# opensensor/thingino-accel

Measured on AMD Instinct MI355X. Metric: images/sec yolov5s_int8 640x640 batch256, higher is better.
Workload: dtype int8

## Files before the change

thingino-accel_amd/csrc/hip/conv_i8.hip:

```cpp
#include "conv_i8_common.hpp"

#ifndef I8M_ABL
#define I8M_ABL 0
#endif
template <int BPX, int BN, int STAGES, int KS = 1, int NW = 4>
__global__ __launch_bounds__(NW * 64) void conv_i8_mfma(const mhip_conv_i8_t p, const long total_pix, const int k64,
                                                         const int8_t *__restrict__ zeros, const unsigned noc,
                                                         const unsigned nblk, const int lg_inc, const unsigned kw_magic,
                                                         const fastdiv_t dhw, const fastdiv_t dow, const int bufmode,
                                                         const unsigned in_bytes) {
    ANAT_BEGIN();
    const bool POW2 = lg_inc >= 0;
    const bool masked = p.kh * p.kw <= 32;
    constexpr int SLICE = (BPX + BN) * BK;
    constexpr int STAGE = KS * SLICE;
    constexpr int NWN = BN == 128 ? 2 : 1;
    constexpr int NWM = NW / NWN;
    constexpr int WPX = BPX / NWM / 16;
    constexpr int WOC = BN / NWN / 16;
    constexpr int XROWS = BPX / NW;
    constexpr int XI = XROWS / 16;
    constexpr int LW = (BN / 16 + NW - 1) / NW;
    constexpr int L = XI + LW;
    static_assert(XI >= 1 && XROWS % 16 == 0, "every wave fetches whole 16-row pieces of the pixel tile");
// ... 713 lines not shown
        if (c < 1.0 || c > 2147483647.0) continue;
        volatile float prod = (float)(int)c * a;
        if (prod == quirk) return 0;
    }
    return 1;
}

extern "C" int mhip_conv_i8_small_c(int in_c, int kw, int out_c) { return in_c <= 4 && kw <= 8 && out_c <= 64; }

extern "C" void mhip_conv_i8_pack_geom(int in_c, int kw, int out_c, int *row_pad, int *oc_pad, int *c_eff) {
    const int small = mhip_conv_i8_small_c(in_c, kw, out_c);
    if (row_pad) *row_pad = small ? 32 : (kw * in_c + 15) & ~15;
    if (oc_pad) *oc_pad = (out_c + 31) & ~31;
    if (c_eff) *c_eff = small ? 4 : in_c;
}

static tune_t g_tune;
static int env_int(const char *name, int dflt) {
    const char *e = getenv(name);
    return e ? atoi(e) : dflt;
}
const tune_t &conv_i8_tune_state() {
    if (!g_tune.init) {
        g_tune.persist = env_int("MARS_HIP_PERSIST", 1);
        g_tune.persist_stages = env_int("MARS_HIP_PSTAGES", 2);
        g_tune.persist_maxk = env_int("MARS_HIP_PERSIST_MAXK", 8);
        g_tune.persist_slots = env_int("MARS_HIP_PSLOTS", 0);
        g_tune.stages = env_int("MARS_HIP_STAGES", 0);
        g_tune.bpx = env_int("MARS_HIP_BPX", 0);
        g_tune.variant = env_int("MARS_HIP_VARIANT", 0);
        g_tune.bufmode = env_int("MARS_HIP_BUFMODE", 1);
        g_tune.wres = env_int("MARS_HIP_WRES", 3);
        g_tune.rgb_direct = env_int("MARS_HIP_RGB_DIRECT", 1);
        g_tune.small_batch = env_int("MARS_HIP_SMALL_BATCH", 1);
        g_tune.rows = env_int("MARS_HIP_ROWS", 1);
        g_tune.few_wgs = env_int("MARS_HIP_FEW_WGS", 256);
        g_tune.patch_ring = env_int("MARS_HIP_PATCH_RING", 0);
        g_tune.patch_lds_kb = env_int("MARS_HIP_PATCH_LDS_KB", 80);
        g_tune.init = 1;
    }
    return g_tune;
}
static inline const tune_t &tune() { return conv_i8_tune_state(); }
static int tune_access(const char *key, int value, int *get) {
    (void)conv_i8_tune_state();
    struct { const char *k; int *v; } tab[] = {{"persist", &g_tune.persist}, {"persist_stages", &g_tune.persist_stages},
                                               {"persist_maxk", &g_tune.persist_maxk}, {"persist_slots", &g_tune.persist_slots}, {"wres", &g_tune.wres}, {"rgb_direct", &g_tune.rgb_direct}, {"small_batch", &g_tune.small_batch},
                                               {"rows", &g_tune.rows}, {"few_wgs", &g_tune.few_wgs}, {"patch_ring", &g_tune.patch_ring}, {"patch_lds_kb", &g_tune.patch_lds_kb}, {"stages", &g_tune.stages}, {"bpx", &g_tune.bpx}, {"variant", &g_tune.variant}, {"bufmode", &g_tune.bufmode}};
    for (auto &e : tab)
        if (key && !strcmp(key, e.k)) {
            if (get) *get = *e.v;
            else *e.v = value;
            return 0;
        }
    return -1;
}
extern "C" int mhip_conv_i8_tune(const char *key, int value) { return tune_access(key, value, nullptr); }
extern "C" int mhip_conv_i8_tune_get(const char *key, int *value) { return value ? tune_access(key, 0, value) : -1; }

static int buf_mode(const mhip_conv_i8_t *p, int k64) {
    if (!tune().bufmode) return 0;
    return p->in_c >= 64 && (p->in_c & (p->in_c - 1)) == 0 && p->kh * p->kw <= 32 && (long)p->kh * p->kw * (p->kw - 1) < 65536 &&
           in_extent_bytes(p) <= 0x7fffffffL && (long)p->oc_pad * k64 <= 0x7fffffffL;
}

template <int BPX, int BN, int STAGES, int KS = 1, int NW = 4>
static int launch_mfma(const mhip_conv_i8_t *p, long total_pix, int k64) {
    const unsigned npt = (unsigned)((total_pix + BPX - 1) / BPX), noc = (unsigned)(p->oc_pad / BN);
    const unsigned nblk = npt * noc;
    const int nks = k64 / BK, nst = nks / KS, used = nst < STAGES ? nst : STAGES;
    if (KS > 1 && (nks % KS) != 0) return -1;
    size_t ring = (size_t)used * KS * (BPX + BN) * BK, tile = (size_t)BPX * (BN + OPAD);
    const size_t lds = BPX * 8 + LUTB + (ring > tile ? ring : tile);
    if (lds > 64 * 1024) {
        static bool attr = false;
        if (!attr && hipFuncSetAttribute((const void *)conv_i8_mfma<BPX, BN, STAGES, KS, NW>, hipFuncAttributeMaxDynamicSharedMemorySize,
                                         (int)(BPX * 8 + LUTB + (size_t)STAGES * KS * (BPX + BN) * BK)) != hipSuccess)
            return mhip_check(hipErrorUnknown, "conv_i8_mfma LDS attribute");
        attr = true;
    }
    int lg = -1;
    if ((p->in_c & (p->in_c - 1)) == 0 && (long)p->kh * p->kw * (p->kw - 1) < 65536) {
        lg = 0;
        while ((1 << lg) < p->in_c) lg++;
    }
    const unsigned magic = ((65536u + (unsigned)p->kw - 1u) / (unsigned)p->kw);
    hipLaunchKernelGGL((conv_i8_mfma<BPX, BN, STAGES, KS, NW>), dim3(nblk), dim3(NW * 64), lds, mhip_stream_native(), *p, total_pix,
                       k64, (const int8_t *)mhip_zero_page(), noc, nblk, lg, magic,
                       make_fastdiv((unsigned)(p->out_h * p->out_w)), make_fastdiv((unsigned)p->out_w),
                       lg >= 0 ? buf_mode(p, k64) : 0, (unsigned)in_extent_bytes(p));
    return mhip_check(hipGetLastError(), "conv_i8_mfma launch");
}


template <int BPX, int BN>
static size_t wres_lds(int k64) { return LUTB + 2 * (size_t)BPX * BK + (size_t)(k64 / BK) * BN * BK; }

template <int BPX, int BN, int STAGES, bool HAS_LUT, bool SEG = false, bool PAIR = false>
static int launch_persist_t(const mhip_conv_i8_t *p, long total_pix, int k64, int lg, unsigned magic,
                            const mhip_conv_i8_t *second = nullptr, int wres = 0) {
    if (BN == 16 && (p->out_c > 16 || p->oc_pad != 32 || (PAIR && (second->out_c > 16 || second->oc_pad != 32)))) return -1;
    const unsigned noc0 = BN == 16 ? 1u : (unsigned)(p->oc_pad / BN);
    const unsigned npt = (unsigned)((total_pix + BPX - 1) / BPX), noc = noc0 + (PAIR ? (BN == 16 ? 1u : (unsigned)(second->oc_pad / BN)) : 0u);
    conv_out_side_t alt;
    memset(&alt, 0, sizeof(alt));
    if (PAIR) {
        alt.out = second->out; alt.out_stride = second->out_stride; alt.w = second->w; alt.bias = second->bias;
        alt.lut = second->lut; alt.lut2 = second->lut2; alt.out_c = second->out_c; alt.relu = second->relu; alt.out_pix_stride = second->out_pix_stride;
        alt.out_ch_off = second->out_ch_off; alt.cs = second->cs;
    }
    if (PAIR) alt.out_bytes = (unsigned)persist_out_bytes(second);
    if (wres && STAGES != 2) return -1;
    const size_t lds = wres ? wres_lds<BPX, BN>(k64) : LUTB + (size_t)STAGES * (BPX + BN) * BK;
    if (wres) {
        static bool attr = false;
        if (!attr && hipFuncSetAttribute((const void *)conv_i8_persist<BPX, BN, STAGES, HAS_LUT, SEG, PAIR>,
                                         hipFuncAttributeMaxDynamicSharedMemorySize, 80 * 1024) != hipSuccess)
            return mhip_check(hipErrorUnknown, "conv_i8_persist LDS attribute");
        attr = true;
        int occ = 0, dev = 0;
        hipDeviceProp_t prop;
        if (hipOccupancyMaxActiveBlocksPerMultiprocessor(&occ, conv_i8_persist<BPX, BN, STAGES, HAS_LUT, SEG, PAIR>, NTHREADS, lds) != hipSuccess ||
            hipGetDevice(&dev) != hipSuccess || hipGetDeviceProperties(&prop, dev) != hipSuccess)
            return mhip_check(hipErrorUnknown, "conv_i8_persist occupancy query");
        unsigned g = (unsigned)((occ > 0 ? occ : 1) * prop.multiProcessorCount) / noc;
        if (tune().persist_slots > 0) g = (unsigned)tune().persist_slots / noc;
        if (g < 1) g = 1;
        if (g > npt) g = npt;
        hipLaunchKernelGGL((conv_i8_persist<BPX, BN, STAGES, HAS_LUT, SEG, PAIR>), dim3(noc * g), dim3(NTHREADS), lds,
                           mhip_stream_native(), *p, (unsigned)total_pix, k64, (const int8_t *)mhip_zero_page(), noc, npt, g, lg,
                           magic, make_fastdiv((unsigned)(p->out_h * p->out_w)), make_fastdiv((unsigned)p->out_w),
                           (unsigned)persist_out_bytes(p), alt, noc0, SEG ? 0 : buf_mode(p, k64), (unsigned)in_extent_bytes(p), 1);
        return mhip_check(hipGetLastError(), "conv_i8_persist (resident weights) launch");
    }
    static int slots = 0;
    if (!slots) {
        int occ = 0, dev = 0;
        hipDeviceProp_t prop;
        if (hipOccupancyMaxActiveBlocksPerMultiprocessor(&occ, conv_i8_persist<BPX, BN, STAGES, HAS_LUT, SEG, PAIR>, NTHREADS, lds) != hipSuccess ||
            hipGetDevice(&dev) != hipSuccess || hipGetDeviceProperties(&prop, dev) != hipSuccess)
            return mhip_check(hipErrorUnknown, "conv_i8_persist occupancy query");
        slots = (occ > 0 ? occ : 1) * prop.multiProcessorCount;
    }
    unsigned ngrp = (unsigned)(tune().persist_slots > 0 ? tune().persist_slots : 4 * slots) / noc;
    if (ngrp < 1) ngrp = 1;
    if (ngrp > npt) ngrp = npt;
    hipLaunchKernelGGL((conv_i8_persist<BPX, BN, STAGES, HAS_LUT, SEG, PAIR>), dim3(noc * ngrp), dim3(NTHREADS), lds,
                       mhip_stream_native(), *p, (unsigned)total_pix, k64, (const int8_t *)mhip_zero_page(), noc, npt, ngrp, lg,
                       magic, make_fastdiv((unsigned)(p->out_h * p->out_w)), make_fastdiv((unsigned)p->out_w),
                       (unsigned)persist_out_bytes(p), alt, noc0, SEG ? 0 : buf_mode(p, k64), (unsigned)in_extent_bytes(p), 0);
    return mhip_check(hipGetLastError(), "conv_i8_persist launch");
}

#define NVARIANTS 20
struct variant_t {
    int persist, bpx, stages, patch, ks2, w8, wres, r128, rows;
};
static int variant_code(const variant_t &v) {
    if (v.rows) return 20;
    if (v.r128) return 17 + v.r128;
    if (v.wres) return v.bpx == 256 ? 15 : 14;
    if (v.w8) return 13;
    if (v.ks2) return 12;
    if (v.patch) return v.patch == 16 ? 10 : (v.patch == 8 ? 9 : 11);
    return 1 + (v.persist ? 1 : 0) + (v.bpx == 256 ? 2 : 0) + (v.stages == 3 ? 4 : 0);
}
static variant_t variant_of(int code) {
    if (code == 20) return variant_t{0, 0, 0, 0, 0, 0, 0, 0, 1};
    if (code == 18 || code == 19) return variant_t{0, 0, 0, 0, 0, 0, 0, code - 17, 0};
    if (code == 14 || code == 15) return variant_t{1, code == 15 ? 256 : 128, 2, 0, 0, 0, 1, 0, 0};
    if (code == 13) return variant_t{0, 256, 3, 0, 0, 1, 0, 0, 0};
    if (code == 12) return variant_t{0, 128, 2, 0, 1, 0, 0, 0, 0};
    if (code >= 9 && code <= 11) return variant_t{0, 0, 0, code == 10 ? 16 : (code == 9 ? 8 : 4), 0, 0, 0, 0, 0};
    if (code > 8 || code == 6 || code == 8) return variant_t{-1, 0, 0, 0, 0, 0, 0, 0, 0};
    const int c = code - 1;
    return variant_t{c & 1, (c & 2) ? 256 : 128, (c & 4) ? 3 : 2, 0, 0, 0, 0, 0, 0};
}

static bool r128_ok(const mhip_conv_i8_t *p) {
    const int C = p->in_c;
    return C >= 128 && (C & (C - 1)) == 0 && p->oc_pad % 128 == 0 && p->kh * p->kw <= 32 && (long)p->kh * p->kw * (p->kw - 1) < 65536 &&
           p->row_pad == p->kw * C && p->nseg <= 1 && in_extent_bytes(p) <= 0x7fffffffL && (long)p->oc_pad * p->kh * p->row_pad <= 0x7fffffffL;
}
template <int BPX, int BN, int NW>
static int launch_r128_t(const mhip_conv_i8_t *p, long total_pix) {
    const int k128 = p->kh * p->row_pad;
    const unsigned npt = (unsigned)((total_pix + BPX - 1) / BPX), noc = (unsigned)(p->oc_pad / BN);
    size_t ring = 2 * (size_t)(BPX + BN) * 128, tile = (size_t)BPX * (BN + OPAD);
    const size_t lds = BPX * 8 + LUTB + (ring > tile ? ring : tile);
    static bool attr = false;
    if (!attr && hipFuncSetAttribute((const void *)conv_i8_r128<BPX, BN, NW>, hipFuncAttributeMaxDynamicSharedMemorySize, (int)lds) != hipSuccess)
        return mhip_check(hipErrorUnknown, "conv_i8_r128 LDS attribute");
    attr = true;
    int lg = 0;
    while ((1 << lg) < p->in_c) lg++;
    const unsigned magic = ((65536u + (unsigned)p->kw - 1u) / (unsigned)p->kw);
    hipLaunchKernelGGL((conv_i8_r128<BPX, BN, NW>), dim3(npt * noc), dim3(NW * 64), lds, mhip_stream_native(), *p, total_pix, k128, noc,
                       npt * noc, lg, magic, make_fastdiv((unsigned)(p->out_h * p->out_w)), make_fastdiv((unsigned)p->out_w),
                       (unsigned)in_extent_bytes(p));
    return mhip_check(hipGetLastError(), "conv_i8_r128 launch");
}
static int launch_r128(const mhip_conv_i8_t *p, long total_pix, int form) {
    if (!r128_ok(p)) return -1;
    return form == 2 ? launch_r128_t<256, 128, 8>(p, total_pix) : launch_r128_t<128, 128, 4>(p, total_pix);
}
static bool seg_valid(const mhip_conv_i8_t *p) {
    if (p->nseg < 2 || p->nseg > 4 || p->kh != 1 || p->kw != 1 || p->stride_h != 1 || p->stride_w != 1 || p->pad_top ||
        p->pad_left || p->in_h != p->out_h || p->in_w != p->out_w)
        return false;
    int c = 0;
    if (p->seg_up && ((p->out_h | p->out_w) & 1)) return false;
    if (p->seg_up >> p->nseg) return false;
    for (int i = 0; i < 4; i++) {
        if (i < p->nseg) {
            if (!p->seg_in[i] || p->seg_c[i] <= 0 || (p->seg_c[i] & 31) || p->seg_c0[i] != c) return false;
            c += p->seg_c[i];
        } else if (p->seg_c0[i] != 0x7fffffff) {
            return false;
        }
    }
    return c == p->in_c;
}
static bool persist_eligible(const mhip_conv_i8_t *p) {
    if (p->add) return false;
    return !p->out_nchw && p->safe && (p->in_c & (p->in_c - 1)) == 0 && p->kh * p->kw <= 32 &&
           (long)p->kh * p->kw * (p->kw - 1) < 65536 && persist_out_bytes(p) <= 0x7fffffffL;
}
static bool wres_default(const mhip_conv_i8_t *p, int nks, int *bpx) {
    if (!tune().wres || p->kh * p->kw != 1 || p->in_c < 64 || p->out_h * p->out_w > 6400) return false;
    const int bn = p->oc_pad % 128 == 0 ? 128 : (p->oc_pad % 64 == 0 ? 64 : 32);
    const int px = (bn == 64 && p->out_h * p->out_w >= 6400) ? 256 : 128;
    if (LUTB + 2 * (size_t)px * BK + (size_t)nks * bn * BK > 80 * 1024) return false;
    *bpx = px;
    return true;
}

static variant_t default_variant(const mhip_conv_i8_t *p, int nks) {
    variant_t v;
    v.patch = 0;
    v.ks2 = 0;
    v.w8 = 0;
    v.wres = 0;
    v.r128 = 0;
    v.rows = 0;
    int ring = 0;
    const long wg_large = ((long)p->frames * p->out_h * p->out_w + 255) / 256 * ((p->oc_pad + 127) / 128);
    const bool few = wg_large < tune().few_wgs && tune().persist && !tune().bpx && !tune().stages && tune().small_batch;
    if (few) {
        if (conv_i8_patch_ok(p, 4, &ring)) {
            v.persist = 0; v.bpx = 0; v.stages = 0; v.patch = 4;
            return v;
        }
        if (nks >= 8 && r128_ok(p)) {
            v.persist = 0; v.bpx = 0; v.stages = 0; v.r128 = 1;
            return v;
        }
        v.bpx = 128;
        v.persist = nks <= tune().persist_maxk && persist_eligible(p);
        if (((p->out_c | p->out_pix_stride | p->out_ch_off) & 15) != 0 && p->nseg <= 1) v.persist = 0;
        v.stages = v.persist ? 2 : 3;
        return v;
    }
    if (tune().persist && !tune().bpx && !tune().stages && tune().rows && p->out_w <= 20 && p->in_c >= 256 && conv_i8_rows_ok(p)) {
        v.persist = 0; v.bpx = 0; v.stages = 0; v.rows = 1;
        return v;
    }
    if (tune().persist && !tune().bpx && !tune().stages) {
        if (conv_i8_patch_ok(p, 16, &ring)) {
            v.persist = 0; v.bpx = 0; v.stages = 0; v.patch = 16;
            return v;
        }
        if (conv_i8_patch_ok(p, 8, &ring) && ring >= 2) {
            v.persist = 0; v.bpx = 0; v.stages = 0; v.patch = 8;
            return v;
        }
    }
    v.bpx = tune().bpx ? tune().bpx : ((p->oc_pad % 128 != 0 && nks <= 2) ? 256 : 128);
    v.persist = tune().persist && nks <= tune().persist_maxk && persist_eligible(p);
    if (((p->out_c | p->out_pix_stride | p->out_ch_off) & 15) != 0 && p->nseg <= 1) v.persist = 0;
    v.stages = v.persist ? 2 : (tune().stages ? tune().stages : (nks <= 4 ? 2 : 3));
    if (v.stages != 3) v.stages = 2;
    if (v.persist && v.stages == 2 && !tune().bpx && wres_default(p, nks, &v.bpx)) v.wres = 1;
    if ((!v.persist || (!v.wres && nks >= 8 && p->nseg <= 1)) && !tune().bpx && !tune().stages && p->oc_pad % 128 == 0 &&
        nks >= (tune().persist_maxk < 8 ? tune().persist_maxk + 1 : 8)) {
        v.persist = 0; v.w8 = 1; v.bpx = 256; v.stages = 3;
    }
    if (p->nseg > 1 && !v.wres && !tune().bpx && nks >= 8) v.bpx = 256;
    return v;
}

template <int BPX, int BN>
static int launch_variant_t(const mhip_conv_i8_t *p, long total_pix, int k64, const variant_t &v) {
    if (v.persist) {
        if (!persist_eligible(p)) return -1;
        int lg = 0;
        while ((1 << lg) < p->in_c) lg++;
        const unsigned magic = ((65536u + (unsigned)p->kw - 1u) / (unsigned)p->kw);
        if (v.wres && wres_lds<BPX, BN>(k64) > 80 * 1024) return -1;
        if (p->nseg > 1)
            return p->lut ? launch_persist_t<BPX, BN, 2, true, true>(p, total_pix, k64, lg, magic, nullptr, v.wres)
                          : launch_persist_t<BPX, BN, 2, false, true>(p, total_pix, k64, lg, magic, nullptr, v.wres);
        if (v.wres)
            return p->lut ? launch_persist_t<BPX, BN, 2, true>(p, total_pix, k64, lg, magic, nullptr, 1)
                          : launch_persist_t<BPX, BN, 2, false>(p, total_pix, k64, lg, magic, nullptr, 1);
        if (v.stages == 2)
            return p->lut ? launch_persist_t<BPX, BN, 2, true>(p, total_pix, k64, lg, magic)
                          : launch_persist_t<BPX, BN, 2, false>(p, total_pix, k64, lg, magic);
        return -1;
    }
    if constexpr (BN == 16) {
        return -1;
    } else {
        if (v.w8) return BN == 128 ? launch_mfma<256, 128, 3, 1, 8>(p, total_pix, k64) : -1;
        if (v.ks2) return BPX == 128 && BN >= 64 ? launch_mfma<128, (BN >= 64 ? BN : 64), 2, 2>(p, total_pix, k64) : -1;
        return v.stages == 2 ? launch_mfma<BPX, BN, 2>(p, total_pix, k64) : launch_mfma<BPX, BN, 3>(p, total_pix, k64);
    }
}
static bool bn16_ok(const mhip_conv_i8_t *p) {
    static const bool off = getenv("MARS_HIP_NO_BN16") != nullptr;
    return !off && p->out_c <= 16 && p->oc_pad == 32 && p->nseg <= 1;
}

static int launch_variant(const mhip_conv_i8_t *p, long total_pix, int k64, const variant_t &v) {
    if (v.persist < 0) return -1;
    if (v.rows) return conv_i8_launch_rows(p);
    if (v.r128) return launch_r128(p, total_pix, v.r128);
    if (v.patch) return conv_i8_launch_patch(p, k64, v.patch);
    const int bn = p->oc_pad % 128 == 0 ? 128 : (p->oc_pad % 64 == 0 ? 64 : 32);
    const bool b16 = v.persist && v.stages == 2 && bn16_ok(p);
    if (v.bpx == 256) {
        if (bn == 128) return launch_variant_t<256, 128>(p, total_pix, k64, v);
        if (bn == 64) return launch_variant_t<256, 64>(p, total_pix, k64, v);
        if (b16) return launch_variant_t<256, 16>(p, total_pix, k64, v);
        return launch_variant_t<256, 32>(p, total_pix, k64, v);
    }
    if (bn == 128) return launch_variant_t<128, 128>(p, total_pix, k64, v);
    if (bn == 64) return launch_variant_t<128, 64>(p, total_pix, k64, v);
    if (b16) return launch_variant_t<128, 16>(p, total_pix, k64, v);
    return launch_variant_t<128, 32>(p, total_pix, k64, v);
}

template <int BPX, int BN>
static int launch_pair_t(const mhip_conv_i8_t *a, const mhip_conv_i8_t *b, long total_pix, int k64, int lg, unsigned magic,
                         int wres) {
    if (a->nseg > 1) return -2;
    return launch_persist_t<BPX, BN, 2, true, false, true>(a, total_pix, k64, lg, magic, b, wres);
}
extern "C" int mhip_conv_i8_pair(const mhip_conv_i8_t *a, const mhip_conv_i8_t *b) {
    if (!a || !b || !tune().persist || tune().variant) return -2;
    if (a->in != b->in || a->in_stride != b->in_stride || a->frames != b->frames || a->in_h != b->in_h || a->in_w != b->in_w ||
        a->in_c != b->in_c || a->out_h != b->out_h || a->out_w != b->out_w || a->kh != b->kh || a->kw != b->kw ||
        a->stride_h != b->stride_h || a->stride_w != b->stride_w || a->pad_top != b->pad_top || a->pad_left != b->pad_left ||
        a->row_pad != b->row_pad || a->nseg != b->nseg || a->seg_up != b->seg_up || !a->lut || !b->lut || a->add || b->add ||
        a->out_nchw || b->out_nchw)
        return -2;
    for (int i = 0; i < a->nseg; i++)
        if (a->seg_in[i] != b->seg_in[i] || a->seg_c[i] != b->seg_c[i] || a->seg_stride[i] != b->seg_stride[i]) return -2;
    if ((a->in_c % 16) != 0 || mhip_conv_i8_small_c(a->in_c, a->kw, a->out_c) || mhip_conv_i8_small_c(b->in_c, b->kw, b->out_c))
        return -2;
    if (a->nseg > 1 && (!seg_valid(a) || !seg_valid(b))) return -2;
    if (!persist_eligible(a) || !persist_eligible(b)) return -2;
    const int bn = a->oc_pad % 128 == 0 ? 128 : (a->oc_pad % 64 == 0 ? 64 : 32);
    const int bnb = b->oc_pad % 128 == 0 ? 128 : (b->oc_pad % 64 == 0 ? 64 : 32);
    if (bn != bnb || !mhip_zero_page()) return -2;
    const long total_pix = (long)a->frames * a->out_h * a->out_w;
    const int k64 = (a->kh * a->row_pad + BK - 1) / BK * BK, nks = k64 / BK;
    if (total_pix <= 0 || total_pix > 0x7fffffffL) return -2;
    int lg = 0;
    while ((1 << lg) < a->in_c) lg++;
    const unsigned magic = ((65536u + (unsigned)a->kw - 1u) / (unsigned)a->kw);
    const variant_t dv = default_variant(a, nks);
    const int bpx = dv.bpx ? dv.bpx : 128, wres = dv.persist && dv.wres && (tune().wres & 2);
    const bool b16 = bn16_ok(a) && bn16_ok(b);
    if (bpx == 256) {
        if (bn == 128) return launch_pair_t<256, 128>(a, b, total_pix, k64, lg, magic, wres);
        if (bn == 64) return launch_pair_t<256, 64>(a, b, total_pix, k64, lg, magic, wres);
        if (b16) return launch_pair_t<256, 16>(a, b, total_pix, k64, lg, magic, wres);
        return launch_pair_t<256, 32>(a, b, total_pix, k64, lg, magic, wres);
    }
    if (bn == 128) return launch_pair_t<128, 128>(a, b, total_pix, k64, lg, magic, wres);
    if (bn == 64) return launch_pair_t<128, 64>(a, b, total_pix, k64, lg, magic, wres);
    if (b16) return launch_pair_t<128, 16>(a, b, total_pix, k64, lg, magic, wres);
    return launch_pair_t<128, 32>(a, b, total_pix, k64, lg, magic, wres);
}

extern "C" int mhip_conv_i8_seg_ok(const mhip_conv_i8_t *p) {
    return p && (p->in_c % 16) == 0 && !mhip_conv_i8_small_c(p->in_c, p->kw, p->out_c) && seg_valid(p) && persist_eligible(p);
}

extern "C" int mhip_conv_i8_variants(const mhip_conv_i8_t *p, int *codes, int max) {
    if (!p || (p->in_c % 16) != 0 || mhip_conv_i8_small_c(p->in_c, p->kw, p->out_c)) return 0;
    const int k64 = (p->kh * p->row_pad + BK - 1) / BK * BK, nks = k64 / BK;
    int n = 0;
    if (p->pre_w) {
        const int first = conv_i8_pre_tile_rows(p);
        for (int th : {first, 16, 8, 4})
            if (th && n < max && conv_i8_patch_ok(p, th, nullptr)) {
                const int code = th == 16 ? 10 : (th == 8 ? 9 : 11);
                bool seen = false;
                for (int i = 0; i < n; i++) seen |= codes[i] == code;
                if (!seen) codes[n++] = code;
            }
        return n;
    }
    if (p->nseg > 1) {
        const int bn = p->oc_pad % 128 == 0 ? 128 : (p->oc_pad % 64 == 0 ? 64 : 32);
        const variant_t dv = default_variant(p, nks);
        const int dflt = dv.persist && dv.wres ? (dv.bpx == 256 ? 15 : 14) : (dv.bpx == 256 ? 4 : 2);
        if (n < max) codes[n++] = dflt;
        if (n < max && dflt != 2) codes[n++] = 2;
        if (n < max && dflt != 4) codes[n++] = 4;
        if (n < max && dflt != 14 && LUTB + 2 * (size_t)128 * BK + (size_t)nks * bn * BK <= 80 * 1024) codes[n++] = 14;
        if (n < max && dflt != 15 && LUTB + 2 * (size_t)256 * BK + (size_t)nks * bn * BK <= 80 * 1024) codes[n++] = 15;
        return n;
    }
    const int dflt = variant_code(default_variant(p, nks));
    if (n < max) codes[n++] = dflt;
    for (int code = 1; code <= NVARIANTS; code++) {
        const variant_t v = variant_of(code);
        if (code == dflt) continue;
        if (v.patch && !conv_i8_patch_ok(p, v.patch, nullptr)) continue;
        if (v.persist && !persist_eligible(p)) continue;
        if (v.ks2 && ((nks & 1) || nks < 4 || p->oc_pad % 64 != 0)) continue;
        if (v.w8 && (p->oc_pad % 128 != 0 || nks < 3)) continue;
        if (v.persist < 0) continue;
        if (v.r128 && !r128_ok(p)) continue;
        if (v.rows && !conv_i8_rows_ok(p)) continue;
        if (v.wres) {
            const int bn = p->oc_pad % 128 == 0 ? 128 : (p->oc_pad % 64 == 0 ? 64 : 32);
            if (LUTB + 2 * (size_t)v.bpx * BK + (size_t)nks * bn * BK > 80 * 1024) continue;
        }
        if (!v.persist && v.stages == 3 && nks <= 2) continue;
        if (n < max) codes[n++] = code;
    }
    return n;
}

template <int BN>
static int launch_generic(const mhip_conv_i8_t *p, long total_pix, int k64) {
    dim3 grid((unsigned)((total_pix + BP - 1) / BP), (unsigned)(p->oc_pad / BN));
    hipLaunchKernelGGL((conv_i8_generic<BN>), grid, dim3(NTHREADS), 0, mhip_stream_native(), *p, total_pix, k64,
                       make_fastdiv((unsigned)(p->out_h * p->out_w)));
    return mhip_check(hipGetLastError(), "conv_i8_generic launch");
}

extern "C" int mhip_conv_i8(const mhip_conv_i8_t *p) {
    if (!p || !p->in || !p->out || !p->w) return -1;
    if (p->out_pix_stride < 0 || p->out_ch_off < 0 || (p->out_nchw && (p->out_pix_stride || p->out_ch_off)) ||
        (p->out_pix_stride && p->out_pix_stride < p->out_ch_off + p->out_c))
        return -1;
    if (p->frames <= 0 || p->in_h <= 0 || p->in_w <= 0 || p->in_c <= 0 || p->out_h <= 0 || p->out_w <= 0 ||
        p->out_c <= 0 || p->kh <= 0 || p->kw <= 0 || p->stride_h < 0 || p->stride_w < 0)
        return -1;
    int row_pad, oc_pad;
    mhip_conv_i8_pack_geom(p->in_c, p->kw, p->out_c, &row_pad, &oc_pad, nullptr);
    if (row_pad != p->row_pad || oc_pad != p->oc_pad) return -1;
    if (p->add && (!p->safe || p->out_nchw || ((p->out_c | p->out_pix_stride | p->out_ch_off) & 15) || (p->in_c % 16) != 0 ||
                   mhip_conv_i8_small_c(p->in_c, p->kw, p->out_c) || p->nseg > 1))
        return -1;
    const long total_pix = (long)p->frames * p->out_h * p->out_w;
    const int k64 = (p->kh * p->row_pad + BK - 1) / BK * BK;
    if (total_pix <= 0 || total_pix > 0x7fffffffL || (total_pix + BP - 1) / BP * (oc_pad / 32) > 0x7fffffffL) return -1;
    if (p->in_planar) {
        if (p->in_planar > 4 || p->in_c != 4 || p->in_w < 4 || p->stride_h < 1 || p->stride_w < 1 || p->add || p->nseg > 1 ||
            !mhip_conv_i8_small_c(p->in_c, p->kw, p->out_c))
            return -2;
        return conv_i8_try_smallc(p, k64);
    }
    if (mhip_conv_i8_small_c(p->in_c, p->kw, p->out_c)) {
        if (p->stride_h >= 1 && p->stride_w >= 1) {
            int rc = conv_i8_try_rgb(p, k64);
            if (rc == -2) rc = conv_i8_try_smallc(p, k64);
            if (rc != -2) return rc;
        }
        if (p->add || p->nseg > 1) return -1;
        if (oc_pad % 64 == 0) return launch_generic<64>(p, total_pix, k64);
        return launch_generic<32>(p, total_pix, k64);
    }
    if (p->pre_w) {
        if (!mhip_zero_page() || !mhip_conv_i8_pre_ok(p)) return -1;
        int th = conv_i8_pre_tile_rows(p);
        const int code = p->variant ? p->variant : tune().variant;
        if (code >= 9 && code <= 11) {
            const int want = code == 10 ? 16 : (code == 9 ? 8 : 4);
            if (conv_i8_patch_ok(p, want, nullptr)) th = want;
        } else if (tune().small_batch && conv_i8_patch_ok(p, 4, nullptr) &&
                   ((long)p->frames * p->out_h * p->out_w + 255) / 256 * ((p->oc_pad + 127) / 128) < 256) {
            th = 4;
        }
        return conv_i8_launch_patch(p, k64, th);
    }
    if ((p->in_c % 16) == 0) {
        if (!mhip_zero_page()) return -1;
        const int nks = k64 / BK;
        if (p->variant < 0 || p->variant > NVARIANTS) return -1;
        int code = p->variant;
        if (p->nseg > 1) {
            if (!seg_valid(p) || !persist_eligible(p)) return -1;
            if (!code && tune().variant) {
                int codes[NVARIANTS];
                const int n = mhip_conv_i8_variants(p, codes, NVARIANTS);
                for (int i = 0; i < n; i++)
                    if (codes[i] == tune().variant) code = codes[i];
            }
            variant_t v = variant_of(code == 4 || code == 14 || code == 15 ? code : 2);
            if (!code) {
                const variant_t dv = default_variant(p, nks);
                v.bpx = dv.bpx ? dv.bpx : 128;
                v.wres = dv.persist && dv.wres;
            }
            return launch_variant(p, total_pix, k64, v);
        }
        if (!code && tune().variant) {
            int codes[NVARIANTS];
            const int n = mhip_conv_i8_variants(p, codes, NVARIANTS);
            for (int i = 0; i < n; i++)
                if (codes[i] == tune().variant) code = codes[i];
        }
        return launch_variant(p, total_pix, k64, code ? variant_of(code) : default_variant(p, nks));
    }
    if (oc_pad % 64 == 0) return launch_generic<64>(p, total_pix, k64);
    return launch_generic<32>(p, total_pix, k64);
}
```

thingino-accel_amd/csrc/hip/conv_i8_common.hpp:

```cpp
#pragma once
#include <hip/hip_runtime.h>
#include <stdint.h>
#include <stdlib.h>
#include <string.h>
#include <type_traits>

#include "../mhip.h"

extern "C" hipStream_t mhip_stream_native(void);
extern "C" int mhip_check(hipError_t e, const char *what);
extern "C" const void *mhip_zero_page(void);

typedef int v4i __attribute__((ext_vector_type(4)));
typedef int v2i __attribute__((ext_vector_type(2)));

#ifdef ANATOMY
struct anat_rec_t {
    unsigned key, wg, hwid, xcc;
    unsigned long long t[4];
};
static __device__ anat_rec_t *g_anat_buf;
static __device__ unsigned g_anat_cap;
#define ANAT_SETTER(NAME)                                                                                                    \
    extern "C" int NAME(void *buf, unsigned cap) {                                                                          \
// ... 250 lines not shown
    constexpr int ROW = BN + OPAD;
    const int lo = p.relu ? 0 : -128;
    const uint8_t *lut128 = slut + 128;
    const int chan = ocw + (lane >> 4) * (4 * WOC);
#pragma unroll
    for (int t = 0; t < WPX; t++) {
        const int prow = pxw + t * 16 + (lane & 15);
        uint32_t pk[WOC];
        int a[WOC * 4];
#pragma unroll
        for (int s = 0; s < WOC; s++)
#pragma unroll
            for (int r = 0; r < 4; r++) a[s * 4 + r] = acc[s][t][r];
        if (DIRECT && SAFE && p.add) {
            const long off = rowoff[prow];
            const bool ok = off >= 0 && oc0 + chan < p.out_c;
            uint32_t xw[WOC];
#pragma unroll
            for (int s = 0; s < WOC; s++) xw[s] = 0;
            if (ok) {
                const int8_t *x = p.add + off + oc0 + chan;
                if (WOC == 4) { const v4i t4 = *(const v4i *)x; xw[0] = t4[0]; xw[1] = t4[1]; xw[WOC > 2 ? 2 : 0] = t4[2]; xw[WOC > 3 ? 3 : 0] = t4[3]; }
                else if (WOC == 2) { const uint2 t2 = *(const uint2 *)x; xw[0] = t2.x; xw[WOC > 1 ? 1 : 0] = t2.y; }
                else xw[0] = *(const uint32_t *)x;
            }
            const add_args_t ga = {p.add_s_conv, p.add_s_other, p.add_inv};
            if (HAS_LUT && LUT0 && p.lut2) requant_pack<WOC * 4, HAS_LUT, true, LUT0, true, true>(a, p.cs, lo, lut128, pk, xw, &ga);
            else requant_pack<WOC * 4, HAS_LUT, true, LUT0, true>(a, p.cs, lo, lut128, pk, xw, &ga);
        } else {
            if (HAS_LUT && LUT0 && SAFE && p.lut2) requant_pack<WOC * 4, HAS_LUT, SAFE, LUT0, false, true>(a, p.cs, lo, lut128, pk);
            else requant_pack<WOC * 4, HAS_LUT, SAFE, LUT0>(a, p.cs, lo, lut128, pk);
        }
        if (DIRECT) {
            const long off = rowoff[prow];
            if (off >= 0 && oc0 + chan < p.out_c) {
                int8_t *d = p.out + off + oc0 + chan;
                if (WOC == 4) *(v4i *)d = (v4i){(int)pk[0], (int)pk[1], (int)pk[2], (int)pk[3]};
                else if (WOC == 2) *(uint2 *)d = make_uint2(pk[0], pk[WOC > 1 ? 1 : 0]);
                else *(uint32_t *)d = pk[0];
            }
        } else {
#pragma unroll
            for (int s = 0; s < WOC; s++) *(uint32_t *)(tile + prow * ROW + chan + s * 4) = pk[s];
        }
    }
    if (DIRECT) return;
    __syncthreads();
    const int ncols = p.out_c - oc0 < BN ? p.out_c - oc0 : BN;
    if (!p.out_nchw && ((p.out_c | p.out_pix_stride | p.out_ch_off) & 15) == 0) {
        constexpr int CPR = BN / 16;
        for (int id = tid; id < BPX * CPR; id += (int)blockDim.x) {
            const int row = id / CPR, c = id - row * CPR;
            const long off = rowoff[row];
            if (off < 0 || c * 16 >= ncols) continue;
            const int8_t *s = tile + row * ROW + c * 16;
            v4i v = {*(const int *)s, *(const int *)(s + 4), *(const int *)(s + 8), *(const int *)(s + 12)};
            *(v4i *)(p.out + off + oc0 + c * 16) = v;
        }
    } else if (!p.out_nchw) {
        constexpr int CPR = BN / 16;
        for (int id = tid; id < BPX * CPR; id += (int)blockDim.x) {
            const int row = id / CPR, c = id - row * CPR;
            const long off = rowoff[row];
            if (off < 0 || c * 16 >= ncols) continue;
            const int8_t *s = tile + row * ROW + c * 16;
            int8_t *d = p.out + off + oc0 + c * 16;
            if (c * 16 + 16 <= ncols) {
                v4i v = {*(const int *)s, *(const int *)(s + 4), *(const int *)(s + 8), *(const int *)(s + 12)};
                __builtin_memcpy(d, &v, 16);
            } else {
                const int rem = ncols - c * 16;
                int o = 0;
                if (rem & 8) { __builtin_memcpy(d, s, 8); o = 8; }
                if (rem & 4) { __builtin_memcpy(d + o, s + o, 4); o += 4; }
                if (rem & 2) { __builtin_memcpy(d + o, s + o, 2); o += 2; }
                if (rem & 1) d[o] = s[o];
            }
        }
    } else {
        for (int id = tid; id < BPX * BN; id += (int)blockDim.x) {
            const int c = id / BPX, row = id - c * BPX;
            const long off = rowoff[row];
            if (off < 0 || c >= ncols) continue;
            p.out[off + (size_t)(oc0 + c) * hw] = tile[row * ROW + c];
        }
    }
}

template <int BPX, int BN, int WPX, int WOC, bool LUT0 = false>
__device__ __forceinline__ void epilogue(const mhip_conv_i8_t &p, v4i (&acc)[WOC][WPX], int8_t *tile, const uint8_t *slut,
                                         const long *rowoff, int oc0, int pxw, int ocw, int hw) {
    const bool direct = !p.out_nchw && ((p.out_c | p.out_pix_stride | p.out_ch_off) & 15) == 0;
#define EPI(L, S, D) epilogue_t<BPX, BN, WPX, WOC, L, S, D, LUT0>(p, acc, tile, slut, rowoff, oc0, pxw, ocw, hw)
    if (direct) {
        if (p.lut) { if (p.safe) EPI(true, true, true); else EPI(true, false, true); }
        else { if (p.safe) EPI(false, true, true); else EPI(false, false, true); }
    } else {
        if (p.lut) { if (p.safe) EPI(true, true, false); else EPI(true, false, false); }
        else { if (p.safe) EPI(false, true, false); else EPI(false, false, false); }
    }
#undef EPI
}

template <int WPX, int WOC>
__device__ __forceinline__ void init_acc(const mhip_conv_i8_t &p, v4i (&acc)[WOC][WPX], int ocbase) {
    const int lane = threadIdx.x & 63;
#pragma unroll
    for (int s = 0; s < WOC; s++) {
        const v4i b = p.bias ? *(const v4i *)(p.bias + ocbase + s * 16 + (lane >> 4) * 4) : (v4i){0, 0, 0, 0};
#pragma unroll
        for (int t = 0; t < WPX; t++) acc[s][t] = b;
    }
}


struct tune_t {
    int init;
    int persist;
    int persist_stages;
    int persist_maxk;
    int persist_slots;
    int stages;
    int bpx;
    int variant;
    int bufmode;
    int small_batch;
    int rgb_direct;
    int wres;
    int few_wgs;
    int rows;
    int patch_ring;
    int patch_lds_kb;
};
const tune_t &conv_i8_tune_state();

extern "C" int mhip_conv_i8_small_c(int in_c, int kw, int out_c);

static inline long in_extent_bytes(const mhip_conv_i8_t *p) {
    return (long)(p->frames - 1) * (long)p->in_stride + (long)p->in_h * p->in_w * p->in_c;
}
static inline long persist_out_bytes(const mhip_conv_i8_t *p) {
    const long pstride = p->out_pix_stride ? p->out_pix_stride : p->out_c;
    return (long)(p->frames - 1) * (long)p->out_stride + (long)p->out_h * p->out_w * pstride;
}
static inline bool conv_i8_direct_rows(const mhip_conv_i8_t *p) {
    return !p->out_nchw && ((p->out_c | p->out_pix_stride | p->out_ch_off) & 15) == 0;
}

bool conv_i8_patch_ok(const mhip_conv_i8_t *p, int th, int *ring);
int conv_i8_launch_patch(const mhip_conv_i8_t *p, int k64, int th);
int conv_i8_pre_tile_rows(const mhip_conv_i8_t *p);
bool conv_i8_rows_ok(const mhip_conv_i8_t *p);
int conv_i8_launch_rows(const mhip_conv_i8_t *p);
int conv_i8_try_rgb(const mhip_conv_i8_t *p, int k64);
int conv_i8_try_smallc(const mhip_conv_i8_t *p, int k64);
```

thingino-accel_amd/csrc/mhip.h:

```cpp
#ifndef MHIP_H
#define MHIP_H

#include <stddef.h>
#include <stdint.h>

#ifdef __cplusplus
extern "C" {
#endif

int mhip_init(int device_hint);
void mhip_shutdown(void);
int mhip_ready(void);
int mhip_device_info(int *cu_count, int *lds_bytes, int *gfx_version, size_t *hbm_bytes);
void *mhip_stream(void);
int mhip_sync(void);
void mhip_select_aux(int on);
void mhip_select_stream(int which);
int mhip_stream_wait(int which, void *ev);
int mhip_event_sync(void *ev);
void *mhip_malloc(size_t bytes);
void mhip_free(void *p);
void *mhip_host_alloc(size_t bytes);
void mhip_host_free(void *p);
int mhip_memset_async(void *dst, int value, size_t bytes);
int mhip_h2d_async(void *dst, const void *src, size_t bytes);
int mhip_d2h_async(void *dst, const void *src, size_t bytes);
int mhip_d2d_async(void *dst, const void *src, size_t bytes);
int mhip_h2d_2d_async(void *dst, size_t dpitch, const void *src, size_t spitch, size_t row_bytes, size_t rows);
int mhip_d2h_2d_async(void *dst, size_t dpitch, const void *src, size_t spitch, size_t row_bytes, size_t rows);
void *mhip_event_create(void);
void *mhip_event_create_sync(void);
void mhip_event_destroy(void *ev);
int mhip_event_record(void *ev);
float mhip_event_elapsed_ms(void *start, void *stop);
const char *mhip_last_error(void);
int mhip_graph_begin(void);
void *mhip_graph_end(int ok);
int mhip_graph_launch(void *exec);
void mhip_graph_destroy(void *exec);

typedef struct {
    const int8_t *in;  size_t in_stride;
    int8_t *out;       size_t out_stride;
    const int8_t *w;
    const int32_t *bias;
    const uint8_t *lut;
    const uint8_t *lut2;
    const int8_t *pre_w;
    const int32_t *pre_bias;
    const uint8_t *pre_lut2;
    float pre_cs;
    const int8_t *w_rgb;
    const int8_t *w_rows;
    int frames;
    int in_h, in_w, in_c;
    int out_h, out_w, out_c;
    int kh, kw, stride_h, stride_w, pad_top, pad_left;
    int row_pad;
    int oc_pad;
    float cs;
    int relu;
    int out_nchw;
    int in_planar;
    int safe;
    int out_pix_stride;
    int out_ch_off;
    int variant;
    const int8_t *add;
    float add_s_conv, add_s_other, add_inv;
    int nseg;
    const int8_t *seg_in[4];
    size_t seg_stride[4];
    int seg_c[4], seg_c0[4];
    int seg_up;
} mhip_conv_i8_t;
int mhip_conv_i8_oc_row(int oc, int oc_pad);
int mhip_conv_i8_pre_ok(const mhip_conv_i8_t *p);
size_t mhip_conv_i8_rgb_pack(int in_c, int kh, int kw, int stride_h, int stride_w, int pad_left, int oc_pad, int k64,
                             const int8_t *packed, int8_t *out);
size_t mhip_conv_i8_rows_pack(int in_c, int kh, int kw, int stride_h, int stride_w, int oc_pad, int k64, int out_w,
                              const int8_t *packed, int8_t *out);
unsigned long mhip_conv_i8_rows_launches(void);
int mhip_conv_i8_is_safe(float cs);
int mhip_conv_i8_lut2_ok(float cs);
int mhip_conv_i8_tune(const char *key, int value);
int mhip_conv_i8_tune_get(const char *key, int *value);
int mhip_conv_i8_variants(const mhip_conv_i8_t *p, int *codes, int max);
int mhip_conv_i8_seg_ok(const mhip_conv_i8_t *p);
int mhip_conv_i8_pair(const mhip_conv_i8_t *a, const mhip_conv_i8_t *b);
int mhip_conv_i8_small_c(int in_c, int kw, int out_c);
void mhip_conv_i8_pack_geom(int in_c, int kw, int out_c, int *row_pad, int *oc_pad, int *c_eff);
int mhip_conv_i8(const mhip_conv_i8_t *p);

typedef struct {
    const float *in;  size_t in_stride;
    float *out;       size_t out_stride;
    const float *w;   const float *bias;
    const void *w_split;
    const void *w_patch;
    int frames;
    int in_h, in_w, in_c, out_h, out_w, out_c;
    int kh, kw, stride_h, stride_w, pad_top, pad_left;
    int silu;
    const float *add; size_t add_stride;
    int use_mfma;
    int k_limit;
    int k_limit_required;
    int in_rec, out_rec;
} mhip_conv_f32_t;
int mhip_conv_f32(const mhip_conv_f32_t *p);
size_t mhip_conv_f32_vcat_pack(int out_c, int in_c, int planes, const float *w, float *out);
int mhip_conv_f32_vcat_head(const mhip_conv_f32_t *p, const float *w_t, const float *const *first, const size_t *first_strides, int n_first, int run_floats);
int mhip_conv_f32_pair(const mhip_conv_f32_t *a, const mhip_conv_f32_t *b);
unsigned long mhip_conv_f32_pair_launches(void);
size_t mhip_conv_f32_split_pack(int out_c, int in_c, int kh, int kw, int stride_w, int planes, const float *w, void *out);
unsigned long mhip_conv_f32_split_launches(void);
int mhip_conv_f32_split_takes(int out_c, int in_c, int kh, int kw, int stride_h, int stride_w, int pad_left, int in_w, int out_w);
size_t mhip_conv_f32_patch_pack(int out_c, int in_c, int kh, int kw, int stride, int pad, int in_h, int in_w, int out_h, int out_w,
                                const float *w, void *out);
size_t mhip_conv_f32_patch_pack2(int out_c, int in_c, int kh, int kw, int stride, int pad, int in_h, int in_w, int out_h, int out_w,
                                 int rec, const float *w, void *out);
int mhip_conv_f32_patch_geom2(int out_c, int in_c, int kh, int kw, int stride, int pad, int in_h, int in_w, int out_h, int out_w,
                              int rec, int *outv, int cap);
unsigned long mhip_conv_f32_prec_launches(void);
unsigned long mhip_conv_f32_recin_launches(void);
int mhip_conv_f32_patch_rec_form(int out_c, int in_c, int kh, int kw, int stride, int pad, int in_h, int in_w, int out_h, int out_w);
int mhip_conv_f32_patch_geom(int out_c, int in_c, int kh, int kw, int stride, int pad, int in_h, int in_w, int out_h, int out_w,
                             int *outv, int cap);
unsigned long mhip_conv_f32_patch_launches(void);
size_t mhip_conv_f32_stem_pack(int out_c, int in_c, int kh, int kw, int stride, int pad, int in_h, int in_w, int out_h, int out_w,
                               const float *w, void *out);
unsigned long mhip_conv_f32_stem_launches(void);
int mhip_conv_f32_mode(int set);

int mhip_lut_i8(const int8_t *in, size_t in_stride, int8_t *out, size_t out_stride, int frames,
                size_t n, const uint8_t *lut_dev);
int mhip_relu_bytes(int8_t *buf, size_t stride, int frames, size_t n);
int mhip_binary_i8(int is_mul, const int8_t *a, size_t a_stride, const int8_t *b, size_t b_stride,
                   int8_t *out, size_t out_stride, int frames, size_t n, float sa, float sb, float inv_so,
                   int out_run, int out_pix_stride, int out_ch_off);
int mhip_sigmoid_f32(const float *in, size_t in_stride, float *out, size_t out_stride, int frames, size_t n);
int mhip_binary_f32(int op , const float *a, size_t a_stride, const float *b,
                    size_t b_stride, float *out, size_t out_stride, int frames, size_t n);
int mhip_relu_f32(const float *in, size_t in_stride, float *out, size_t out_stride, int frames,
                  size_t n, float alpha);
int mhip_batchnorm_i8(const int8_t *in, size_t in_stride, int8_t *out, size_t out_stride, int frames,
                      int n, int c, int hw, const float *s, const float *b, float in_scale, float out_scale);
int mhip_batchnorm_f32(const float *in, size_t in_stride, float *out, size_t out_stride, int frames,
                       int n, int c, int hw, const float *s, const float *b);

int mhip_maxpool_i8(const int8_t *in, size_t in_stride, int8_t *out, size_t out_stride, int frames,
                    int in_h, int in_w, int ch, int out_h, int out_w, int kh, int kw, int sh, int sw,
                    int out_pix_stride, int out_ch_off);
int mhip_pool_chain_i8(const int8_t *in, size_t in_stride, int8_t *const *outs, const size_t *out_strides, int n,
                       int frames, int h, int w, int ch, int kh, int kw);
int mhip_unpad_rows(const void *src, void *dst, size_t rows, int width, int pitch);
int mhip_concat_slice(const int8_t *in, size_t in_stride, int8_t *out, size_t out_stride, int frames,
                      int out_h, int out_w, int in_c, int out_c, int ch_off);
int mhip_concat_nchwq(const int8_t *const *ins, const size_t *in_strides, const int *in_c, int n, int8_t *out, size_t out_stride,
                      int frames, int out_c, int H, int W, int rows_only );
int mhip_upsample_nchwq(const int8_t *in, size_t in_stride, int Ci, int Hi, int Wi, int8_t *out, size_t out_stride, int Co, int Ho, int Wo,
                        int frames, int qih, int qiw, int qch, int qoh, int qow, int sh, int sw);
int mhip_maxpool_nchwq(const int8_t *in, size_t in_stride, int8_t *out, size_t out_stride, int frames, int C, int H, int W, int kh, int kw);
int mhip_upsample_i8(const int8_t *in, size_t in_stride, int8_t *out, size_t out_stride, int frames,
                     int in_h, int in_w, int ch, int out_h, int out_w, int scale_h, int scale_w,
                     int out_pix_stride, int out_ch_off);
int mhip_nchw_to_nhwc_pad(const int8_t *in, size_t in_stride, int8_t *out, size_t out_stride,
                          int frames, int c, int hw, int c_pad);

typedef struct {
    const int8_t *pred[4]; size_t stride[4]; int npred[4];
    int pix_c[4], pix_stride[4];
    const float *lut[4];
    int mono[4];
    int nseg;
    int frames;
    float nms_thresh;
    void *dets;
    int *counts;
    int *raw_counts;
    int do_nms;
} mhip_detect_t;
int mhip_detect(const mhip_detect_t *p);
int mhip_nms_only(void *dets_dev, int *count_dev, int n, float thresh);

typedef struct {
    const uint8_t *rgb; size_t rgb_stride;
    int8_t *out;        size_t out_stride;
    int frames, w, h, tw, th, nhwc;
    int nw, nh, px, py;
    const int *xstart, *xsrc; const float *xw;
    const int *ystart, *ysrc; const float *yw;
    int max_cols, max_rows;
    int n_xtaps;
    int max_ytaps;
    int form;
} mhip_letterbox_t;
int mhip_letterbox(const mhip_letterbox_t *p);

#ifdef __cplusplus
}
#endif
#endif
```

Baseline: 57080.

## Add deep 3x3 stride-1 conv kernel with LDS input patch reuse

Adds a new int8 conv kernel for 3x3 stride-1 convolutions with 128 or 256 input channels on 20- or 40-wide maps. It loads a padded input patch for a 256-pixel tile into LDS once per 64-channel chunk and reuses it across all nine taps, while weights stream through a four-stage ring. The kernel is selected by default ahead of the patch and generic paths and can be disabled with an environment variable. It adds 512-thread blocks with more LDS use and hand-placed barriers and waitcnts, which may limit occupancy.

```diff
diff --git a/thingino-accel_amd/csrc/hip/conv_i8.hip b/thingino-accel_amd/csrc/hip/conv_i8.hip
--- a/thingino-accel_amd/csrc/hip/conv_i8.hip
+++ b/thingino-accel_amd/csrc/hip/conv_i8.hip
@@ -889,11 +889,12 @@
     return mhip_check(hipGetLastError(), "conv_i8_persist launch");
 }
 
-#define NVARIANTS 20
+#define NVARIANTS 21
 struct variant_t {
-    int persist, bpx, stages, patch, ks2, w8, wres, r128, rows;
+    int persist, bpx, stages, patch, ks2, w8, wres, r128, rows, deep;
 };
 static int variant_code(const variant_t &v) {
+    if (v.deep) return 21;
     if (v.rows) return 20;
     if (v.r128) return 17 + v.r128;
     if (v.wres) return v.bpx == 256 ? 15 : 14;
@@ -903,6 +904,7 @@
     return 1 + (v.persist ? 1 : 0) + (v.bpx == 256 ? 2 : 0) + (v.stages == 3 ? 4 : 0);
 }
 static variant_t variant_of(int code) {
+    if (code == 21) return variant_t{0, 0, 0, 0, 0, 0, 0, 0, 0, 1};
     if (code == 20) return variant_t{0, 0, 0, 0, 0, 0, 0, 0, 1};
     if (code == 18 || code == 19) return variant_t{0, 0, 0, 0, 0, 0, 0, code - 17, 0};
     if (code == 14 || code == 15) return variant_t{1, code == 15 ? 256 : 128, 2, 0, 0, 0, 1, 0, 0};
@@ -972,6 +974,11 @@
     return true;
 }
 
+static bool deep3_on() {
+    static const bool off = getenv("MARS_HIP_NO_DEEP3") != nullptr && atoi(getenv("MARS_HIP_NO_DEEP3")) != 0;
+    return !off;
+}
+
 static variant_t default_variant(const mhip_conv_i8_t *p, int nks) {
     variant_t v;
     v.patch = 0;
@@ -980,6 +987,7 @@
     v.wres = 0;
     v.r128 = 0;
     v.rows = 0;
+    v.deep = 0;
     int ring = 0;
     const long wg_large = ((long)p->frames * p->out_h * p->out_w + 255) / 256 * ((p->oc_pad + 127) / 128);
     const bool few = wg_large < tune().few_wgs && tune().persist && !tune().bpx && !tune().stages && tune().small_batch;
@@ -1000,6 +1008,10 @@
     }
     if (tune().persist && !tune().bpx && !tune().stages && tune().rows && p->out_w <= 20 && p->in_c >= 256 && conv_i8_rows_ok(p)) {
         v.persist = 0; v.bpx = 0; v.stages = 0; v.rows = 1;
+        return v;
+    }
+    if (tune().persist && !tune().bpx && !tune().stages && deep3_on() && conv_i8_deep_ok(p)) {
+        v.persist = 0; v.bpx = 0; v.stages = 0; v.deep = 1;
         return v;
     }
     if (tune().persist && !tune().bpx && !tune().stages) {
@@ -1060,6 +1072,7 @@
 
 static int launch_variant(const mhip_conv_i8_t *p, long total_pix, int k64, const variant_t &v) {
     if (v.persist < 0) return -1;
+    if (v.deep) return conv_i8_launch_deep(p);
     if (v.rows) return conv_i8_launch_rows(p);
     if (v.r128) return launch_r128(p, total_pix, v.r128);
     if (v.patch) return conv_i8_launch_patch(p, k64, v.patch);
@@ -1163,6 +1176,7 @@
         if (v.persist < 0) continue;
         if (v.r128 && !r128_ok(p)) continue;
         if (v.rows && !conv_i8_rows_ok(p)) continue;
+        if (v.deep && !conv_i8_deep_ok(p)) continue;
         if (v.wres) {
             const int bn = p->oc_pad % 128 == 0 ? 128 : (p->oc_pad % 64 == 0 ? 64 : 32);
             if (LUTB + 2 * (size_t)v.bpx * BK + (size_t)nks * bn * BK > 80 * 1024) continue;
diff --git a/thingino-accel_amd/csrc/hip/conv_i8_common.hpp b/thingino-accel_amd/csrc/hip/conv_i8_common.hpp
--- a/thingino-accel_amd/csrc/hip/conv_i8_common.hpp
+++ b/thingino-accel_amd/csrc/hip/conv_i8_common.hpp
@@ -426,5 +426,7 @@
 int conv_i8_pre_tile_rows(const mhip_conv_i8_t *p);
 bool conv_i8_rows_ok(const mhip_conv_i8_t *p);
 int conv_i8_launch_rows(const mhip_conv_i8_t *p);
+bool conv_i8_deep_ok(const mhip_conv_i8_t *p);
+int conv_i8_launch_deep(const mhip_conv_i8_t *p);
 int conv_i8_try_rgb(const mhip_conv_i8_t *p, int k64);
 int conv_i8_try_smallc(const mhip_conv_i8_t *p, int k64);
diff --git a/thingino-accel_amd/csrc/hip/conv_i8_deep.hip b/thingino-accel_amd/csrc/hip/conv_i8_deep.hip
--- /dev/null
+++ b/thingino-accel_amd/csrc/hip/conv_i8_deep.hip
@@ -0,0 +1,207 @@
+#include "conv_i8_common.hpp"
+
+#define DP_NPX 256
+#define DP_BN 128
+#define DP_RING 4
+#define DP_STAGE (DP_BN * BK)
+#define DP_NDWMAX 5
+#define DP_ROWOFF LUTB
+#define DP_ROWTAB (DP_ROWOFF + DP_NPX * 8)
+#define DP_RINGB (DP_ROWTAB + 512)
+#define DP_PATCH (DP_RINGB + DP_RING * DP_STAGE)
+
+struct deep_args_t {
+    int W, H, C;
+    int prmax;
+    int npieces;
+    unsigned noc, nblk;
+    unsigned npix;
+    unsigned in_bytes, w_bytes;
+    fastdiv_t dW, dH, dH1, dhw;
+};
+
+template <int PWP, int NCH>
+__global__ __launch_bounds__(512) __attribute__((amdgpu_waves_per_eu(4, 4))) void conv_i8_deep(const mhip_conv_i8_t p,
+                                                                                             const deep_args_t a) {
+    ANAT_BEGIN();
+    extern __shared__ __attribute__((aligned(16))) int8_t dynlds[];
+    uint8_t *slut = (uint8_t *)dynlds;
+    lds_base_must_be_zero(dynlds);
+    long *rowoff = (long *)(dynlds + DP_ROWOFF);
+    int *rowtab = (int *)(dynlds + DP_ROWTAB);
+    int8_t *ring = dynlds + DP_RINGB;
+    constexpr int NK = NCH * 9;
+
+    const int tid = threadIdx.x, lane = tid & 63;
+    const int wv = __builtin_amdgcn_readfirstlane(tid >> 6);
+    const int wm = wv & 3, wn = wv >> 2;
+    const int frow = lane & 15, fchunk = lane >> 4;
+    const unsigned id = xcd_remap(blockIdx.x, a.nblk);
+    const unsigned t = id / a.noc, ot = id - t * a.noc;
+    const int oc0 = (int)ot * DP_BN;
+    const int W = a.W, H = a.H, C = a.C;
+    const unsigned P0 = t * (unsigned)DP_NPX;
+    const unsigned g0 = fdiv(P0, a.dW), f0 = fdiv(g0, a.dH), y0 = g0 - f0 * (unsigned)H;
+
+    v4i acc[4][4];
+    init_acc<4, 4>(p, acc, oc0 + wn * 64);
+    if (p.lut2) { if (tid < 128) ((uint32_t *)slut)[tid] = ((const uint32_t *)p.lut2)[tid]; }
+    else if (p.lut && tid < 64) ((uint32_t *)slut)[tid] = ((const uint32_t *)p.lut)[tid];
+    fill_rowoff<DP_NPX>(p, rowoff, [=](int row) { long q = (long)P0 + row; return q < (long)a.npix ? q : -1L; },
+                        (unsigned)(H * W), a.dhw);
+    if (tid >= 256 && tid - 256 < a.prmax) {
+        const unsigned r = (unsigned)(tid - 256);
+        const unsigned v = f0 * (unsigned)(H + 1) + y0 + r;
+        const unsigned f = fdiv(v, a.dH1);
+        const int iy = (int)(v - f * (unsigned)(H + 1)) - 1;
+        rowtab[r] = iy >= 0 && f < (unsigned)p.frames ? (int)(f * (unsigned)p.in_stride) + iy * W * C : -1;
+    }
+    const __amdgpu_buffer_rsrc_t xrs = __builtin_amdgcn_make_buffer_rsrc((void *)p.in, 0, (int)a.in_bytes, 0x00020000);
+    const __amdgpu_buffer_rsrc_t wrs = __builtin_amdgcn_make_buffer_rsrc((void *)p.w_rows, 0, (int)a.w_bytes, 0x00020000);
+    const int wvoff = wv * 1024 + lane * 16;
+    const int wblk0 = (int)ot * NK;
+    __syncthreads();
+
+    auto issue_patch = [&](int ch) __attribute__((always_inline)) {
+#pragma unroll
+        for (int j = 0; j < DP_NDWMAX; j++) {
+            if (j * 8 + wv >= a.npieces) continue;
+            const unsigned phys = (unsigned)((j * 8 + wv) * 64 + lane);
+            const unsigned U = phys ^ ((phys >> 3) & 2u);
+            const unsigned pix = U >> 2, c16 = U & 3u;
+            const unsigned prow = pix / (unsigned)PWP, pcol = pix - prow * (unsigned)PWP;
+            const int ro = prow < (unsigned)a.prmax ? rowtab[prow] : -1;
+            const bool ok = ro >= 0 && pcol >= 1u && pcol <= (unsigned)W;
+            const int voff = ok ? ro + ((int)pcol - 1) * C + (int)c16 * 16 : -1;
+            blds16(xrs, voff, ch * 64, dynlds + DP_PATCH + (j * 8 + wv) * 1024);
+        }
+    };
+    auto issue_w = [&](int s) __attribute__((always_inline)) {
+        blds16(wrs, wvoff, (wblk0 + s) * DP_STAGE, ring + (s % DP_RING) * DP_STAGE + wv * 1024);
+    };
+    unsigned pxu[4];
+#pragma unroll
+    for (int u = 0; u < 4; u++) {
+        const unsigned P = P0 + (unsigned)(wm * 64 + u * 16 + frow);
+        const unsigned g = fdiv(P, a.dW), x = P - g * (unsigned)W;
+        const unsigned tr = g - g0, cross = fdiv(y0 + tr, a.dH);
+        pxu[u] = (tr + cross) * (unsigned)PWP + x;
+    }
+    issue_patch(0);
+#pragma unroll
+    for (int s = 0; s < DP_RING - 1; s++) issue_w(s);
+    ANAT_NOW(1);
+#pragma unroll
+    for (int s = 0; s < NK; s++) {
+        const int tap = s % 9, ky = tap / 3, kx = tap - ky * 3;
+        if (NK - 1 - s >= 2) wait_vmcnt<2>();
+        else if (NK - 1 - s == 1) wait_vmcnt<1>();
+        else wait_vmcnt<0>();
+        __builtin_amdgcn_sched_barrier(0);
+        asm volatile("s_waitcnt lgkmcnt(0)\n\ts_barrier" ::: "memory");
+        __builtin_amdgcn_sched_barrier(0);
+        if (tap == 0 && s > 0) {
+            issue_patch(s / 9);
+            if (s + DP_RING - 1 < NK) issue_w(s + DP_RING - 1);
+            if (s + DP_RING - 1 < NK) wait_vmcnt<1>();
+            else wait_vmcnt<0>();
+            __builtin_amdgcn_sched_barrier(0);
+            __builtin_amdgcn_s_barrier();
+            __builtin_amdgcn_sched_barrier(0);
+        } else if (s + DP_RING - 1 < NK) {
+            issue_w(s + DP_RING - 1);
+        }
+        asm volatile("" ::: "memory");
+        v4i xb[4], wa[4];
+        const int8_t *ws = ring + (s % DP_RING) * DP_STAGE;
+#pragma unroll
+        for (int q = 0; q < 4; q++) wa[q] = *(const v4i *)(ws + lds_off(wn * 64 + q * 16 + frow, fchunk));
+#pragma unroll
+        for (int u = 0; u < 4; u++) {
+            const unsigned px = pxu[u] + (unsigned)kx;
+            xb[u] = *(const v4i *)(dynlds + DP_PATCH + (int)(px * 64u) + ((fchunk * 16) ^ (int)((px & 4u) << 3)) + ky * (PWP * 64));
+        }
+#pragma unroll
+        for (int q = 0; q < 4; q++)
+#pragma unroll
+            for (int u = 0; u < 4; u++) acc[q][u] = __builtin_amdgcn_mfma_i32_16x16x64_i8(wa[q], xb[u], acc[q][u], 0, 0, 0);
+    }
+    ANAT_NOW(2);
+    __syncthreads();
+    epilogue<DP_NPX, DP_BN, 4, 4, true>(p, acc, ring, slut, rowoff, oc0, wm * 64, wn * 64, H * W);
+    ANAT_END(p);
+}
+ANAT_SETTER(mhip_anatomy_set_deep)
+
+struct deep_geom_t {
+    deep_args_t a;
+    int pwp, nch;
+    size_t lds;
+};
+static bool deep_geom(const mhip_conv_i8_t *p, deep_geom_t *g) {
+    const int C = p->in_c, W = p->out_w, H = p->out_h;
+    if (!p->w_rows || p->kh != 3 || p->kw != 3 || p->stride_h != 1 || p->stride_w != 1 || p->pad_top != 1 || p->pad_left != 1 ||
+        p->in_h != H || p->in_w != W || (C != 128 && C != 256) || p->oc_pad % DP_BN != 0 || p->row_pad != 3 * C || p->nseg > 1 ||
+        p->pre_w || p->in_planar)
+        return false;
+    if (p->add && (!p->safe || !conv_i8_direct_rows(p))) return false;
+    if (W != 20 && W != 40) return false;
+    if (in_extent_bytes(p) > 0x7fffffffL || persist_out_bytes(p) > 0x7fffffffL || (long)p->oc_pad * 9 * C > 0x7fffffffL) return false;
+    deep_args_t &a = g->a;
+    a.W = W; a.H = H; a.C = C;
+    g->nch = C / 64;
+    g->pwp = (W + 2 + 7) & ~7;
+    const int maxrows = (DP_NPX + W - 2) / W + 1;
+    a.prmax = maxrows + 2 + (maxrows + H - 2) / H;
+    if (a.prmax > 128) return false;
+    const long units = (long)a.prmax * g->pwp * 4;
+    a.npieces = (int)((units + 63) / 64);
+    if (a.npieces > 8 * DP_NDWMAX) return false;
+    g->lds = DP_PATCH + (size_t)a.npieces * 1024;
+    if (g->lds > 80 * 1024 || (size_t)DP_NPX * (DP_BN + OPAD) > g->lds - DP_RINGB) return false;
+    const long npix = (long)p->frames * H * W;
+    if (npix > 0x3fffffffL) return false;
+    a.npix = (unsigned)npix;
+    a.noc = (unsigned)(p->oc_pad / DP_BN);
+    const long nblk = (npix + DP_NPX - 1) / DP_NPX * a.noc;
+    if (nblk > 0x7fffffffL) return false;
+    a.nblk = (unsigned)nblk;
+    a.in_bytes = (unsigned)in_extent_bytes(p);
+    a.w_bytes = (unsigned)((long)p->oc_pad * 9 * C);
+    a.dW = make_fastdiv((unsigned)W);
+    a.dH = make_fastdiv((unsigned)H);
+    a.dH1 = make_fastdiv((unsigned)(H + 1));
+    a.dhw = make_fastdiv((unsigned)(H * W));
+    return true;
+}
+
+bool conv_i8_deep_ok(const mhip_conv_i8_t *p) {
+    deep_geom_t g;
+    return deep_geom(p, &g);
+}
+extern "C" int mhip_conv_i8_deep_ok(const mhip_conv_i8_t *p) { return p && conv_i8_deep_ok(p) ? 1 : 0; }
+
+template <int PWP, int NCH>
+static int launch_deep_t(const mhip_conv_i8_t *p, const deep_geom_t &g) {
+    auto kern = conv_i8_deep<PWP, NCH>;
+    static bool attr = false;
+    if (!attr && hipFuncSetAttribute((const void *)kern, hipFuncAttributeMaxDynamicSharedMemorySize, 80 * 1024) != hipSuccess)
+        return mhip_check(hipErrorUnknown, "conv_i8_deep attribute");
+    attr = true;
+    hipLaunchKernelGGL(kern, dim3(g.a.nblk), dim3(512), g.lds, mhip_stream_native(), *p, g.a);
+    return mhip_check(hipGetLastError(), "conv_i8_deep launch");
+}
+
+static unsigned long g_deep_launches = 0;
+extern "C" unsigned long mhip_conv_i8_deep_launches(void) { return g_deep_launches; }
+
+int conv_i8_launch_deep(const mhip_conv_i8_t *p) {
+    deep_geom_t g;
+    if (!deep_geom(p, &g)) return -1;
+    g_deep_launches++;
+    if (g.pwp == 48 && g.nch == 2) return launch_deep_t<48, 2>(p, g);
+    if (g.pwp == 48 && g.nch == 4) return launch_deep_t<48, 4>(p, g);
+    if (g.pwp == 24 && g.nch == 2) return launch_deep_t<24, 2>(p, g);
+    if (g.pwp == 24 && g.nch == 4) return launch_deep_t<24, 4>(p, g);
+    return -1;
+}
diff --git a/thingino-accel_amd/csrc/mhip.h b/thingino-accel_amd/csrc/mhip.h
--- a/thingino-accel_amd/csrc/mhip.h
+++ b/thingino-accel_amd/csrc/mhip.h
@@ -81,6 +81,8 @@
 size_t mhip_conv_i8_rows_pack(int in_c, int kh, int kw, int stride_h, int stride_w, int oc_pad, int k64, int out_w,
                               const int8_t *packed, int8_t *out);
 unsigned long mhip_conv_i8_rows_launches(void);
+int mhip_conv_i8_deep_ok(const mhip_conv_i8_t *p);
+unsigned long mhip_conv_i8_deep_launches(void);
 int mhip_conv_i8_is_safe(float cs);
 int mhip_conv_i8_lut2_ok(float cs);
 int mhip_conv_i8_tune(const char *key, int value);
```

Measured after the change: 57750, median of 6. 1.2% higher.
